# jby1993/SelfReconCode

Measured on AMD Instinct MI355X. Metric: train.py-equivalent iterations/sec (540x540, 2048 rays/frame x 3 frames per GPU; coarse stage at Adam lr 0.0001), higher is better.
Workload: dtype f32

## Files before the change

### include/selfrecon_hip.h

```cpp
#ifndef SELFRECON_HIP_H_
#define SELFRECON_HIP_H_
#include <stdint.h>

#ifdef __cplusplus
extern "C" {
#endif

#define SR_OK 0
#define SR_EINVAL (-1)
#define SR_ELAUNCH (-2)
#define SR_ENOSPC (-3)

int sr_abi_version(void);
const char* sr_build_arch(void);
const char* sr_build_digest(void);

int sr_minv3x3_fwd_f32(const float* ms, float* invs, uint8_t* checks, int64_t n, void* stream);
int sr_minv3x3_fwd_f64(const double* ms, double* invs, uint8_t* checks, int64_t n, void* stream);
int sr_minv3x3_bwd_f32(const float* grads, const float* invs, float* outs, int64_t n, void* stream);
int sr_minv3x3_bwd_f64(const double* grads, const double* invs, double* outs, int64_t n, void* stream);

typedef struct {
  int64_t size[5];
  int64_t stride[5];
// ... 64 lines not shown
  const float* Z; int64_t ldz;
  const float* A; int64_t lda;
  float* dW; int64_t lddw;
  float* partial;
  int32_t R, N, K, splits, accumulate;
  float* db; float* db_partial; int32_t group;
} sr_gemm_tn_args;
int64_t sr_mlp_gemm_tn_workspace_floats(int32_t R, int32_t N, int64_t lddw, int32_t* host_splits_out);
int sr_mlp_gemm_tn(const sr_gemm_tn_args* host_args, void* stream);
#define SR_TN_GROUP_MAX 12
typedef struct {
  int32_t n;
  sr_gemm_tn_args p[SR_TN_GROUP_MAX];
} sr_gemm_tn_group_args;
int sr_mlp_gemm_tn_group(const sr_gemm_tn_group_args* host_args, void* stream);

int sr_pe_embed(const float* x, int64_t P, int32_t L, const float* band_weights, const float* extra, int64_t ldextra,
                int32_t E, const int64_t* extra_index , int32_t group, float* out, int64_t ldo, void* stream);
int sr_pe_embed_bwd(const float* x, int64_t P, int32_t L, const float* band_weights, int32_t group, const float* gA0,
                    int64_t ldg, float* xbar, void* stream);

typedef struct {
  const float* p; const float* tp; int64_t P;
  const float* A; const float* trans; int32_t nframes;
  const int64_t* batch_inds; int64_t points_per_frame;
  const float* vol; int32_t D, H, W;
  float bmin[3], bmax[3];
  float* y;
  float* jac;
} sr_lbs_args;
// ... 195 lines not shown
```

### selfreconcode_amd/_lib.py

```python
import ctypes
import os
import torch

from .build import LIB

_i64, _vp, _int = ctypes.c_int64, ctypes.c_void_p, ctypes.c_int


class SrTensor5(ctypes.Structure):
    _fields_ = [("size", _i64 * 5), ("stride", _i64 * 5)]


class SrGemmArgs(ctypes.Structure):
    _fields_ = [("A", _vp), ("lda", _i64), ("B", _vp), ("ldb", _i64), ("C", _vp), ("ldc", _i64),
                ("M", ctypes.c_int32), ("N", ctypes.c_int32), ("K", ctypes.c_int32), ("bias", _vp),
                ("group", ctypes.c_int32), ("act", ctypes.c_int32), ("mode", ctypes.c_int32), ("out_scale", ctypes.c_float),
                ("aux", _vp), ("ldaux", _i64), ("naux_fwd", ctypes.c_int32), ("nact_bwd", ctypes.c_int32),
                ("aux_scale", ctypes.c_float)]


class SrGemmTnArgs(ctypes.Structure):
    _fields_ = [("Z", _vp), ("ldz", _i64), ("A", _vp), ("lda", _i64), ("dW", _vp), ("lddw", _i64), ("partial", _vp),
                ("R", ctypes.c_int32), ("N", ctypes.c_int32), ("K", ctypes.c_int32), ("splits", ctypes.c_int32),
                ("accumulate", ctypes.c_int32), ("db", _vp), ("db_partial", _vp), ("group", ctypes.c_int32)]
# ... 124 lines not shown
    "sr_gridsample3d_fwd_f64": [_vp, _T5, _vp, _T5, _vp, _T5, _vp],
    "sr_gridsample3d_bwd_f32": [_vp, _T5, _vp, _T5, _vp, _T5, _vp, _T5, _vp, _vp],
    "sr_gridsample3d_bwd_f64": [_vp, _T5, _vp, _T5, _vp, _T5, _vp, _T5, _vp, _vp],
    "sr_gridsample3d_dbwd_f32": [_vp, _T5, _vp, _T5, _vp, _T5, _vp, _T5, _vp, _T5, _vp, _T5, _vp, _vp, _vp],
    "sr_gridsample3d_dbwd_f64": [_vp, _T5, _vp, _T5, _vp, _T5, _vp, _T5, _vp, _T5, _vp, _T5, _vp, _vp, _vp],
    "sr_mlp_gemm_nt": [_vp, _vp],
    "sr_mlp_gemm_nt_tile": [ctypes.c_int32, ctypes.c_int32, _vp, _vp],
    "sr_mlp_chain": [_vp, _vp],
    "sr_refine_init": [_vp, _vp],
    "sr_refine_embed": [_vp, ctypes.c_int32, _vp],
    "sr_refine_mid": [_vp, ctypes.c_int32, ctypes.c_int32, _vp],
    "sr_refine_finish": [_vp, ctypes.c_int32, _vp],
    "sr_mlp_gemm_tn_workspace_floats": [ctypes.c_int32, ctypes.c_int32, _i64, _vp],
    "sr_mlp_gemm_tn": [_vp, _vp],
    "sr_mlp_gemm_tn_group": [_vp, _vp],
    "sr_lbs_chain_fwd": [_vp, ctypes.c_int32, _vp, _vp, _vp, _vp, _vp, _vp],
    "sr_lbs_chain_bwd": [_vp, ctypes.c_int32, _vp, _vp, _vp, _vp, _vp, _vp, _vp],
    "sr_lbs_fwd": [_vp, _vp],
    "sr_lbs_bwd_workspace_floats": [_i64, ctypes.c_int32],
    "sr_lbs_bwd": [_vp, _vp, _vp, _vp, _vp, _vp, _vp],
    "sr_lbs_jac_bwd": [_vp, _vp, _vp, _vp, _vp, _vp, _vp, _vp],
    "sr_newton_update": [_vp, _vp],
    "sr_newton_prepare": [_vp, _vp],
    "sr_newton_apply": [_vp, _vp],
    "sr_mc_workspace_bytes": [ctypes.c_int32, ctypes.c_int32, ctypes.c_int32],
    "sr_mc_count": [_vp, ctypes.c_int32, ctypes.c_int32, ctypes.c_int32, ctypes.c_float, _vp, _vp, _vp],
    "sr_mc_emit": [_vp, ctypes.c_int32, ctypes.c_int32, ctypes.c_int32, ctypes.c_float, _vp] + [ctypes.c_float] * 6 + [_vp, _vp, _vp],
    "sr_rows_pad": [_vp, _i64, ctypes.c_int32, _vp, _i64, ctypes.c_int32, _i64, ctypes.c_int32, _vp, _i64, ctypes.c_int32, _vp],
    "sr_rows_frame_sum_workspace_floats": [_i64, ctypes.c_int32, ctypes.c_int32],
    "sr_rows_frame_sum": [_vp, _i64, _i64, ctypes.c_int32, _vp, ctypes.c_int32, _vp, _vp, _vp],
# ... 46 lines not shown
    "sr_texture_fill_workspace_bytes": [ctypes.c_int32],
    "sr_texture_fill": [_vp, _vp, _vp, ctypes.c_int32, ctypes.c_int32, _vp, _vp, _vp],
    "sr_lbsw_knn_blend": [_vp, _vp, _i64] + [ctypes.c_int32] * 5 + [_vp, _vp, ctypes.c_int32, _vp, _vp],
    "sr_lbsw_smooth": [_vp, _vp] + [ctypes.c_int32] * 4 + [_vp],
    "sr_smpl_shape": [_vp, _vp, _vp, ctypes.c_int32, ctypes.c_int32, _i64, _vp, _vp],
    "sr_smpl_regress_workspace_floats": [ctypes.c_int32, _i64, ctypes.c_int32],
    "sr_smpl_regress": [_vp, _vp, ctypes.c_int32, _i64, ctypes.c_int32, _vp, _vp, _vp],
    "sr_smpl_pose": [_vp, _vp, _vp, _vp, ctypes.c_int32, _vp, _vp, _vp, _vp],
    "sr_smpl_skin": [_vp, _i64, _vp, _vp, _vp, _vp, ctypes.c_int32, _i64, _vp, _vp],
    "sr_meshreg_workspace_bytes": [_i64, _i64],
    "sr_meshreg_fwd": [_vp, _i64, _vp, _vp, _i64, _vp, _i64, ctypes.c_int32, ctypes.c_float] + [_vp] * 6,
    "sr_meshreg_bwd": [_i64, _vp, _vp, _i64, _vp, _vp, _i64] + [_vp] * 8,
    "sr_pe_embed_bwd": [_vp, _i64, ctypes.c_int32, _vp, ctypes.c_int32, _vp, _i64, _vp, _vp],
    "sr_pe_embed": [_vp, _i64, ctypes.c_int32, _vp, _vp, _i64, ctypes.c_int32, _vp, ctypes.c_int32, _vp, _i64, _vp],
}
_RESTYPE = {"sr_rows_frame_sum_workspace_floats": _i64, "sr_lbs_bwd_workspace_floats": _i64, "sr_mlp_gemm_tn_workspace_floats": _i64, "sr_mc_workspace_bytes": _i64, "sr_points_silhouette_workspace_bytes": _i64,
            "sr_texture_fill_workspace_bytes": _i64, "sr_meshreg_workspace_bytes": _i64, "sr_smpl_regress_workspace_floats": _i64}

_fn = {}
for _name, _args in SIGNATURES.items():
    try:
        _f = getattr(_lib, _name)
    except AttributeError as e:
        raise ImportError(f"{LIB} does not export {_name}; rebuild it") from e
    _f.argtypes = _args
    _f.restype = _RESTYPE.get(_name, _int)
    _fn[_name] = _f
_lib.sr_abi_version.restype = _int
_lib.sr_build_arch.restype = ctypes.c_char_p
_lib.sr_build_digest.restype = ctypes.c_char_p

# ... 61 lines not shown
        t = t.float()
    return t if t.is_contiguous() else t.contiguous()


def i64c(t):
    t = t.detach()
    if t.dtype != torch.int64:
        t = t.long()
    return t if t.is_contiguous() else t.contiguous()


_raw_stream = getattr(torch._C, "_cuda_getCurrentRawStream", None)


def stream_of(t):
    if _raw_stream is not None and t.device.index is not None:
        return _raw_stream(t.device.index)
    return torch.cuda.current_stream(t.device).cuda_stream


class _NoContext:
    def __enter__(self):
        return self

    def __exit__(self, *exc):
        return False


_NO_CONTEXT = _NoContext()


def on_device(dev):
    if dev.index is not None and dev.index == torch.cuda.current_device():
# ... 18 lines not shown
```

### selfreconcode_amd/csrc/mlp_gemm.hip

```cpp
#include "sr_common.h"
#include <stdlib.h>
#include <type_traits>

typedef float f32x16 __attribute__((ext_vector_type(16)));
typedef float f32x4 __attribute__((ext_vector_type(4)));
typedef int i32x4 __attribute__((ext_vector_type(4)));

__device__ __forceinline__ __amdgpu_buffer_rsrc_t sr_make_rsrc(const void* base, int64_t bytes) {
  return __builtin_amdgcn_make_buffer_rsrc(const_cast<void*>(base), 0, (int)(bytes < 0xFFFFFFFFll ? bytes : 0xFFFFFFFFll), 0x00020000);
}
__device__ __forceinline__ f32x4 sr_buffer_load16(__amdgpu_buffer_rsrc_t rsrc, uint32_t lane_off, uint32_t scalar_off) {
  return __builtin_bit_cast(f32x4, __builtin_amdgcn_raw_buffer_load_b128(rsrc, (int)lane_off, (int)scalar_off, 0));
}

namespace {

constexpr int BK = 32;
constexpr int LDSP = BK + 4;

__device__ __forceinline__ float fast_exp(float x) { return __builtin_amdgcn_exp2f(x * 1.4426950408889634f); }
__device__ __forceinline__ float fast_log(float x) { return __builtin_amdgcn_logf(x) * 0.6931471805599453f; }
__device__ __forceinline__ float softplus100(float z) {
  const float t = z * 100.0f;
  const float e = fast_exp(fminf(t, 20.0f));
// ... 586 lines not shown
  int blocks[SR_TN_GROUP_MAX];
  int rows_per_split[SR_TN_GROUP_MAX];
  sr_gemm_tn_args p[SR_TN_GROUP_MAX];
};
__global__ __launch_bounds__(256) __attribute__((amdgpu_waves_per_eu(2))) void gemm_tn_group_kernel(TnGroup G) {
  extern __shared__ __attribute__((aligned(16))) float tn_smem[];
  int i = 0;
  while (i + 1 < G.n && (int)blockIdx.x >= G.first[i + 1]) ++i;
  const int bid = blockIdx.x - G.first[i];
  if (bid >= G.blocks[i]) return;
  gemm_tn_body<128, 128>(G.p[i], G.rows_per_split[i], bid, G.blocks[i], tn_smem);
}

static inline bool tn_narrow(int N, int64_t K) { return K <= 64 && N >= 256; }

__device__ __forceinline__ void slab_reduce_body(const float* __restrict__ partial, float* __restrict__ dW, int N,
                                                 int K, int64_t lddw, int splits, int accumulate,
                                                 const float* __restrict__ db_partial, float* __restrict__ db, int bid, int nblocks) {
  const int64_t total = (int64_t)N * lddw;
  const int64_t quads = total >> 2;
  const int64_t all = quads + (db ? N : 0);
  const f32x4* __restrict__ p4 = reinterpret_cast<const f32x4*>(partial);
  f32x4* __restrict__ d4 = reinterpret_cast<f32x4*>(dW);
  for (int64_t i = (int64_t)bid * blockDim.x + threadIdx.x; i < all; i += (int64_t)nblocks * blockDim.x) {
    if (i < quads) {
      const int col = (int)((i << 2) % lddw);
      f32x4 s = {0.f, 0.f, 0.f, 0.f};
      if (col < K) {
        const f32x4* src = p4 + i;
        int p = 0;
        for (; p + 8 <= splits; p += 8) {
          f32x4 v[8];
#pragma unroll
          for (int j = 0; j < 8; ++j) v[j] = src[(int64_t)(p + j) * quads];
#pragma unroll
          for (int j = 0; j < 8; ++j) s += v[j];
        }
        for (; p < splits; ++p) s += src[(int64_t)p * quads];
        if (col + 1 >= K) s.y = 0.f;
        if (col + 2 >= K) s.z = 0.f;
        if (col + 3 >= K) s.w = 0.f;
      }
      f32x4 o = {0.f, 0.f, 0.f, 0.f};
      if (accumulate) o = d4[i];
      d4[i] = o + s;
    } else {
      const int n = (int)(i - quads);
      float s = 0.f;
      for (int p = 0; p < splits; ++p) s += db_partial[(int64_t)p * N + n];
      db[n] = (accumulate ? db[n] : 0.f) + s;
    }
  }
}

__global__ __launch_bounds__(256) void slab_reduce_kernel(const float* __restrict__ partial, float* __restrict__ dW, int N,
                                                           int K, int64_t lddw, int splits, int accumulate,
                                                           const float* __restrict__ db_partial, float* __restrict__ db) {
  slab_reduce_body(partial, dW, N, K, lddw, splits, accumulate, db_partial, db, blockIdx.x, gridDim.x);
}

__global__ __launch_bounds__(256) void slab_reduce_group_kernel(TnGroup G) {
  int i = 0;
  while (i + 1 < G.n && (int)blockIdx.x >= G.first[i + 1]) ++i;
  const int bid = blockIdx.x - G.first[i];
  if (bid >= G.blocks[i]) return;
  const sr_gemm_tn_args& g = G.p[i];
  slab_reduce_body(g.partial, g.dW, g.N, g.K, g.lddw, g.R > 0 ? g.splits : 0, g.accumulate, g.db_partial, g.db, bid, G.blocks[i]);
}

}

static void nt_tile_choice(int M, int ncols, int* bm, int* bn) {
  auto cost = [&](int tm, int tn, double eff) {
    const int64_t wgs = sr_cdiv(M, tm) * sr_cdiv(ncols, tn);
    return (double)sr_cdiv(wgs, 256) * tm * tn / eff;
  };
  if (ncols <= 32) {
    const double c[3] = {cost(32, 32, 0.6), cost(64, 32, 0.8), cost(256, 32, 1.0)};
    *bn = 32;
    if (c[0] < c[1] && c[0] < c[2]) *bm = 32;
    else if (c[1] < c[2]) *bm = 64;
    else *bm = 256;
// ... 91 lines not shown
  }
  return sr_launch_status();
}

int64_t sr_mlp_gemm_tn_workspace_floats(int32_t R, int32_t N, int64_t lddw, int32_t* splits_out) {
  const int tiles = tn_narrow(N, lddw) ? (int)sr_cdiv(N, 256) : (int)(sr_cdiv(N, 128) * sr_cdiv(lddw, 128));
  const int target = 512;
  int splits = (int)sr_cdiv(target, tiles);
  const int max_splits = (int)sr_cdiv(R, 384);
  if (splits > max_splits) splits = max_splits;
  if (splits < 1) splits = 1;
  if (splits_out) *splits_out = splits;
  return (int64_t)splits * N * lddw;
}

int sr_mlp_gemm_tn(const sr_gemm_tn_args* a, void* stream) {
  if (!a || !a->dW || !a->partial || a->R < 0 || a->N <= 0 || a->K <= 0 || a->splits < 1) return SR_EINVAL;
  if (a->R > 0 && (!a->Z || !a->A)) return SR_EINVAL;
  if ((a->ldz & 3) || (a->lda & 3) || ((uintptr_t)a->Z & 15) || ((uintptr_t)a->A & 15) || a->lddw < a->K) return SR_EINVAL;
  if ((a->lddw & 3) || ((uintptr_t)a->dW & 15) || ((uintptr_t)a->partial & 15)) return SR_EINVAL;
  if ((a->db != nullptr) != (a->db_partial != nullptr) || (a->db && a->group < 1)) return SR_EINVAL;
  const bool narrow = tn_narrow(a->N, a->lddw);
  const int tiles = narrow ? (int)sr_cdiv(a->N, 256) : (int)(sr_cdiv(a->N, 128) * sr_cdiv(a->K, 128));
  int rows_per_split = (int)sr_cdiv(a->R, a->splits);
  rows_per_split = (int)(sr_cdiv(rows_per_split, TBR) * TBR);
  if (a->R > 0) {
    using Narrow = TnCfg<256, 64>;
    using Square = TnCfg<128, 128>;
    if (narrow)
      hipLaunchKernelGGL((gemm_tn_kernel<256, 64>), dim3(tiles * a->splits), dim3(256), Narrow::kLdsFloats * sizeof(float), (hipStream_t)stream, *a,
                         rows_per_split);
    else
      hipLaunchKernelGGL((gemm_tn_kernel<128, 128>), dim3(tiles * a->splits), dim3(256), Square::kLdsFloats * sizeof(float), (hipStream_t)stream, *a,
                         rows_per_split);
  }
  const int64_t total = (int64_t)a->N * a->lddw / 4 + (a->db ? a->N : 0);
  hipLaunchKernelGGL(slab_reduce_kernel, dim3(sr_stream_grid(total, 256)), dim3(256), 0, (hipStream_t)stream, a->partial, a->dW,
                     a->N, a->K, a->lddw, a->R > 0 ? a->splits : 0, a->accumulate, a->db_partial, a->db);
  return sr_launch_status();
}

static int tn_check(const sr_gemm_tn_args* a) {
  if (!a || !a->dW || !a->partial || a->R < 0 || a->N <= 0 || a->K <= 0 || a->splits < 1) return SR_EINVAL;
  if (a->R > 0 && (!a->Z || !a->A)) return SR_EINVAL;
  if ((a->ldz & 3) || (a->lda & 3) || ((uintptr_t)a->Z & 15) || ((uintptr_t)a->A & 15) || a->lddw < a->K) return SR_EINVAL;
  if ((a->lddw & 3) || ((uintptr_t)a->dW & 15) || ((uintptr_t)a->partial & 15)) return SR_EINVAL;
  if ((a->db != nullptr) != (a->db_partial != nullptr) || (a->db && a->group < 1)) return SR_EINVAL;
  return SR_OK;
}

int sr_mlp_gemm_tn_group(const sr_gemm_tn_group_args* a, void* stream) {
  if (!a || a->n < 1 || a->n > SR_TN_GROUP_MAX) return SR_EINVAL;
  TnGroup G, Rd;
  G.n = Rd.n = a->n;
  int nb = 0, nr = 0;
  bool any_rows = false;
  for (int i = 0; i < a->n; ++i) {
    const sr_gemm_tn_args& p = a->p[i];
    const int rc = tn_check(&p);
    if (rc != SR_OK) return rc;
    if (tn_narrow(p.N, p.lddw)) return SR_EINVAL;
    const int tiles = (int)(sr_cdiv(p.N, 128) * sr_cdiv(p.K, 128));
    int rows_per_split = (int)sr_cdiv(p.R, p.splits);
    rows_per_split = (int)(sr_cdiv(rows_per_split, TBR) * TBR);
    G.p[i] = Rd.p[i] = p;
    G.rows_per_split[i] = Rd.rows_per_split[i] = rows_per_split;
    G.first[i] = nb; G.blocks[i] = p.R > 0 ? tiles * p.splits : 0;
    nb += (int)(sr_cdiv(G.blocks[i], 8) * 8);
    const int64_t total = (int64_t)p.N * p.lddw / 4 + (p.db ? p.N : 0);
    Rd.first[i] = nr; Rd.blocks[i] = sr_stream_grid(total, 256);
    nr += Rd.blocks[i];
    any_rows = any_rows || p.R > 0;
  }
  G.first[a->n] = nb; Rd.first[a->n] = nr;
  using Square = TnCfg<128, 128>;
  if (any_rows && nb > 0)
    hipLaunchKernelGGL(gemm_tn_group_kernel, dim3(nb), dim3(256), Square::kLdsFloats * sizeof(float), (hipStream_t)stream, G);
  hipLaunchKernelGGL(slab_reduce_group_kernel, dim3(nr), dim3(256), 0, (hipStream_t)stream, Rd);
  return sr_launch_status();
}
}

namespace {
__global__ __launch_bounds__(256) void pe_embed_kernel(const float* __restrict__ x, int64_t P, int L, const float* __restrict__ w,
                                                        const float* __restrict__ extra, int64_t ldextra, int E,
                                                        const int64_t* __restrict__ extra_index, int group,
                                                        float* __restrict__ out, int64_t ldo) {
  const int width = 3 + 6 * L + E;
  const int64_t total = P * ldo;
  for (int64_t i = (int64_t)blockIdx.x * blockDim.x + threadIdx.x; i < total; i += (int64_t)gridDim.x * blockDim.x) {
    const int64_t p = i / ldo;
    const int c = (int)(i % ldo);
    float v = 0.f, t3[3] = {0.f, 0.f, 0.f};
// ... 68 lines not shown
```

### selfreconcode_amd/mlp_engine.py

```python
import collections
import contextlib
import ctypes
import math
import os
import weakref
import torch

from . import _lib

ACT_NONE, ACT_SOFTPLUS100, ACT_RELU = 0, 1, 2
EPI_FWD, EPI_BWD = 0, 1

TN_SIDE_STREAM = True
GROUP_TN_BELOW = 16384
DEBUG_TN_DELAY_MS = int(os.environ.get("SR_DEBUG_TN_DELAY_MS", "0"))
_TN_STREAMS = {}
_TN_PENDING = set()
_DELAY_FLAG = {}

DEFERRED_PARAM_GRADS = False

_PACK_CACHE = {}
_ENTRY_BY_PTR = {}

_INPUT_GRADS_ONLY = False


def pad4(n):
    return (n + 3) // 4 * 4


# ... 22 lines not shown
                layers.append(LayerSpec(k, n - K0, ACT_SOFTPLUS100, 1.0 / math.sqrt(2.0), nfill=K0))
            else:
                layers.append(LayerSpec(k, n, ACT_NONE if last else ACT_SOFTPLUS100))
            k = n
        return MLPSpec(layers, K0)

    @staticmethod
    def relu_mlp(K0, widths):
        layers, k = [], K0
        for i, n in enumerate(widths):
            layers.append(LayerSpec(k, n, ACT_NONE if i == len(widths) - 1 else ACT_RELU))
            k = n
        return MLPSpec(layers, K0)


_GemmRecord = collections.namedtuple("_GemmRecord", "e0 e1 flop rows overlap N K mode group")


class _GemmProfile:

    def __init__(self):
        self.overlap = False
        self.reset(enabled=False)

    def reset(self, enabled, reserve=0):
        self.enabled = enabled
        self.records, self.chains, self.pool = [], [], []
        for _ in range(reserve if enabled else 0):
            e0, e1 = torch.cuda.Event(enable_timing=True), torch.cuda.Event(enable_timing=True)
            e0.record(); e1.record()
            self.pool.append((e0, e1))

    def pair(self):
        return self.pool.pop() if self.pool else (torch.cuda.Event(enable_timing=True), torch.cuda.Event(enable_timing=True))

    def launch(self, name, args, stream, timed=True, what=None, marks=None):
        if not (timed and self.enabled):
            _lib.call(name, ctypes.byref(args), stream)
            return
        e0, e1 = self.pair()
        e0.record()
        _lib.call(name, ctypes.byref(args), stream)
        e1.record()
        if marks is not None:
            marks.append((e0, e1) + what)
        else:
            rows, N, K, mode, group = what
            self.records.append(_GemmRecord(e0, e1, 2.0 * rows * N * K, rows, self.overlap, N, K, mode, group))

    def summary(self):
        if not self.records:
            return {"tflops": 0.0, "launches": 0, "avg_us": 0.0, "avg_flop": 0.0}
        torch.cuda.synchronize()
        for marks, live, overlap in self.chains:
            lv = live.tolist()
            for e0, e1, phase, fpr in marks:
                self.records.append(_GemmRecord(e0, e1, fpr * lv[phase], lv[phase], overlap, 0, 0, "chain", 1))
        self.chains = []
        times = [r.e0.elapsed_time(r.e1) for r in self.records]

        def rate(sel):
            f = sum(r.flop for r, t, k in zip(self.records, times, sel) if k)
            ms = sum(t for t, k in zip(times, sel) if k)
            n = sum(1 for k in sel if k)
            return (f / (ms * 1e-3) / 1e12 if ms > 0 else 0.0), n, (ms * 1e3 / n if n else 0.0), (f / n if n else 0.0)

        nt = [r.mode != "tn" for r in self.records]
        alone = [k and not r.overlap for k, r in zip(nt, self.records)]
        tf, n, us, fl = rate(alone)
        tf_all, n_all, us_all, _ = rate(nt)
        tf_big, n_big, _, _ = rate([a and r.rows >= 65536 for a, r in zip(alone, self.records)])
        tf_tn, n_tn, us_tn, _ = rate([not k for k in nt])
        self._times = times
        f_nt = float(sum(r.flop for r, k in zip(self.records, nt) if k))
        f_tn = float(sum(r.flop for r, k in zip(self.records, nt) if not k))
        return {"tflops": round(tf, 3), "launches": n, "avg_us": round(us, 3), "avg_flop": round(fl, 1), "tflops_large": round(tf_big, 3),
                "launches_large": n_big, "tflops_all": round(tf_all, 3), "launches_all": n_all, "avg_us_all": round(us_all, 3),
                "avg_flop_all": round(f_nt / max(n_all, 1), 1), "flops_total": f_nt, "flops_total_tn": f_tn,
                "tflops_tn": round(tf_tn, 3), "launches_tn": n_tn, "avg_us_tn": round(us_tn, 3)}

    def by_shape(self):
        if not self.records:
            return []
        times = getattr(self, "_times", None) or [r.e0.elapsed_time(r.e1) for r in self.records]
        acc = {}
        for r, t in zip(self.records, times):
            a = acc.setdefault((r.rows, r.N, r.K, r.mode, r.group, bool(r.overlap)), [0, 0.0, 0.0])
            a[0] += 1; a[1] += r.flop; a[2] += t
        rows = [{"M": k[0], "N": k[1], "K": k[2], "mode": k[3], "group": k[4], "overlap": k[5], "launches": v[0], "flop": v[1], "ms": round(v[2], 4),
                 "tflops": round(v[1] / (v[2] * 1e-3) / 1e12, 2) if v[2] > 0 else 0.0} for k, v in acc.items()]
        rows.sort(key=lambda r: -r["ms"])
        return rows


PROFILE = _GemmProfile()


def set_gemm_args(a, A, B, C, M, N, K, bias, group, act, mode, out_scale=1.0, aux=None, naux_fwd=0, nact_bwd=0, aux_scale=1.0, pitches=None):
    lda, ldb, ldc, ldaux = pitches or (A.stride(0), B.stride(0), C.stride(0), 0 if aux is None else aux.stride(0))
# ... 14 lines not shown
_TnProblem = collections.namedtuple("_TnProblem", "Z ldz A lda R N K lddw group dW db accumulate")


def _tn_workspace(R, N, lddw):
    splits = ctypes.c_int32(0)
    ws = _lib.raw("sr_mlp_gemm_tn_workspace_floats")(R, N, lddw, ctypes.byref(splits))
    return max(int(ws), 1), splits.value


def _set_tn_args(a, Z, ldz, A, lda, R, N, K, lddw, group, dW, db, accumulate, partial, ws, splits):
    a.Z, a.ldz, a.A, a.lda, a.dW, a.lddw, a.partial = Z.data_ptr(), ldz, A.data_ptr(), lda, dW.data_ptr(), lddw, partial
    a.R, a.N, a.K, a.splits, a.accumulate = R, N, K, splits, 1 if accumulate else 0
    a.db, a.db_partial, a.group = db.data_ptr(), partial + 4 * ws, group


def _gemm_tn(Z, ldz, A, lda, R, N, K, lddw, group=1, dW=None, db=None, accumulate=False):
    ws, splits = _tn_workspace(R, N, lddw)
    if dW is None:
        dW = torch.empty((N, lddw), dtype=torch.float32, device=Z.device)
    partial = torch.empty((ws + splits * N,), dtype=torch.float32, device=Z.device)
    if db is None:
        db = torch.empty((N,), dtype=torch.float32, device=Z.device)
    a = _lib.SrGemmTnArgs()
    _set_tn_args(a, Z, ldz, A, lda, R, N, K, lddw, group, dW, db, accumulate, partial.data_ptr(), ws, splits)
    PROFILE.launch("sr_mlp_gemm_tn", a, _lib.stream_of(Z), R >= 128 and N > 32, (R, N, K, "tn", group))
    return dW, db


def _tn_is_narrow(N, lddw):
    return lddw <= 64 and N >= 256


def _gemm_tn_group(problems):
    problems = [_TnProblem(*p) for p in problems]
    g = _lib.SrGemmTnGroupArgs()
    g.n = len(problems)
    sizes, total = [], 0
    for p in problems:
        ws, splits = _tn_workspace(p.R, p.N, p.lddw)
        sizes.append((ws, splits, total))
        total += (ws + splits * p.N + 3) // 4 * 4
    partial = torch.empty((total,), dtype=torch.float32, device=problems[0].Z.device)
    for a, p, (ws, splits, off) in zip(g.p, problems, sizes):
        _set_tn_args(a, *p, partial.data_ptr() + 4 * off, ws, splits)
    _lib.call("sr_mlp_gemm_tn_group", ctypes.byref(g), _lib.stream_of(partial))


def _debug_delay(device, ms):
    f = _DELAY_FLAG.get(str(device))
# ... 6 lines not shown
    key = str(device)
    st = _TN_STREAMS.get(key)
    if st is None:
        st = _TN_STREAMS[key] = torch.cuda.Stream(device=device)
    return st


def _launch_on_tn_stream(device, problems):
    main, side = torch.cuda.current_stream(device), _tn_stream(device)
    ready = torch.cuda.Event()
    ready.record(main)
    side.wait_event(ready)
    with torch.cuda.stream(side):
        if DEBUG_TN_DELAY_MS:
            _debug_delay(device, DEBUG_TN_DELAY_MS)
        if len(problems) == 1:
            p = problems[0]
            _gemm_tn(*p[:9], dW=p.dW, db=p.db, accumulate=p.accumulate)
        else:
            _gemm_tn_group(problems)
    for p in problems:
        p.Z.record_stream(side); p.A.record_stream(side)
    _TN_PENDING.add(str(device))


def join_weight_gradient_stream():
    for key in list(_TN_PENDING):
        st = _TN_STREAMS[key]
        torch.cuda.current_stream(st.device).wait_stream(st)
    _TN_PENDING.clear()


def _check_mat(t, name):
    if t.dtype != torch.float32 or not t.is_cuda or t.dim() != 2 or t.stride(1) != 1 or (t.stride(0) % 4) or (t.data_ptr() % 16):
        raise RuntimeError(f"mlp_engine: {name} must be a GPU fp32 matrix with unit column stride, row pitch % 4 == 0 "
                           f"and 16-byte alignment (got {tuple(t.shape)}, strides {t.stride()}, {t.dtype}, {t.device})")


def _bias_segments(b0, R, group):
    if b0 is None or b0.dim() != 2:
        return None
# ... 47 lines not shown
    if TN_SIDE_STREAM and not PROFILE.enabled:
        return _DW_SIDE, sink
    return _DW_SINK, sink


def reverse(spec, A0, WTs, acts, Ybar, group, need_input_grad=True, need_param_grad=True, Ws=None, bs=None):
    _check_mat(Ybar, "Ybar")
    R = A0.shape[0]
    nl = len(spec.layers)
    dWs, dbs = [None] * nl, [None] * nl
    A0bar_extra = None
    Zbar = Ybar
    A0bar = None
    seg = _bias_segments(bs[0], R, group) if bs is not None else None
    grouped = [] if (0 < R < GROUP_TN_BELOW and TN_SIDE_STREAM and not PROFILE.enabled) else None
    with _lib.on_device(A0.device):
        for l in range(nl - 1, -1, -1):
            L = spec.layers[l]
            X = A0 if l == 0 else acts[l - 1]
            if need_param_grad:
                route, sink = _weight_gradient_route(l, L, Ws, bs, seg, grouped)
                if sink is not None:
                    p = _TnProblem(Zbar, Zbar.stride(0), X, X.stride(0), R, L.N, L.K, pad4(L.K), group, *sink)
                    if route == _DW_GROUPED:
                        grouped.append(p)
                    elif route == _DW_SIDE:
                        _launch_on_tn_stream(A0.device, [p])
                    else:
                        _gemm_tn(*p[:9], dW=p.dW, db=p.db, accumulate=p.accumulate)
                elif route == _DW_SEGMENTED:
                    S, rs = seg
                    dWs[0] = torch.empty((L.N, pad4(L.K)), dtype=torch.float32, device=A0.device)
                    dbs[0] = torch.zeros((S, L.N), dtype=torch.float32, device=A0.device)
                    for s in range(S):
                        _gemm_tn(Zbar[s * rs:(s + 1) * rs], Zbar.stride(0), X[s * rs:(s + 1) * rs], X.stride(0), rs, L.N, L.K, pad4(L.K), group,
                                 dW=dWs[0], db=dbs[0][s], accumulate=s > 0)
                else:
                    dWs[l], dbs[l] = _gemm_tn(Zbar, Zbar.stride(0), X, X.stride(0), R, L.N, L.K, pad4(L.K), group)
            if l > 0:
                Pv = spec.layers[l - 1]
                Znew = torch.empty((R, pad4(L.K)), dtype=torch.float32, device=A0.device)
                _gemm_nt(Zbar, Zbar.stride(0), WTs[l], WTs[l].stride(0), Znew, Znew.stride(0), R, L.K, L.N, None, group, Pv.act,
                         EPI_BWD, out_scale=Pv.out_scale, aux=acts[l - 1], ldaux=acts[l - 1].stride(0), nact_bwd=Pv.N,
                         aux_scale=Pv.out_scale)
                if Pv.nfill and need_input_grad:
                    A0bar_extra = Znew[:, Pv.N:Pv.N + Pv.nfill]
                Zbar = Znew
            elif need_input_grad:
                A0bar = torch.empty((R, pad4(L.K)), dtype=torch.float32, device=A0.device)
                _gemm_nt(Zbar, Zbar.stride(0), WTs[0], WTs[0].stride(0), A0bar, A0bar.stride(0), R, L.K, L.N, None, 1, ACT_NONE,
                         EPI_FWD)
                if A0bar_extra is not None:
                    A0bar[:, :A0bar_extra.shape[1]] += A0bar_extra
        if grouped:
            _launch_on_tn_stream(A0.device, grouped)
    return A0bar, dWs, dbs


def transpose_padded(W, K):
    N = W.shape[0]
    WT = torch.zeros((K, pad4(N)), dtype=W.dtype, device=W.device)
    WT[:, :N] = W[:, :K].t()
    return WT


def pad_cols(t, width):
    if t.shape[1] == width and t.is_contiguous():
        return t
    return torch.nn.functional.pad(t, (0, width - t.shape[1]))

# ... 390 lines not shown
```

Measured before the change: 23.49.

## Defer weight-gradient slab reductions and batch them into one multi-problem reduce kernel

```diff
diff --git a/include/selfrecon_hip.h b/include/selfrecon_hip.h
--- a/include/selfrecon_hip.h
+++ b/include/selfrecon_hip.h
@@ -102,6 +102,10 @@
   sr_gemm_tn_args p[SR_TN_GROUP_MAX];
 } sr_gemm_tn_group_args;
 int sr_mlp_gemm_tn_group(const sr_gemm_tn_group_args* host_args, void* stream);
+int sr_mlp_gemm_tn_tiles(const sr_gemm_tn_args* host_problems, int32_t n, void* stream);
+int64_t sr_mlp_slab_reduce_many_table_bytes(int32_t n);
+int sr_mlp_slab_reduce_many(const sr_gemm_tn_args* host_problems, int32_t n, void* table_host, void* table_dev, int64_t table_bytes,
+                            void* stream);
 
 int sr_pe_embed(const float* x, int64_t P, int32_t L, const float* band_weights, const float* extra, int64_t ldextra,
                 int32_t E, const int64_t* extra_index , int32_t group, float* out, int64_t ldo, void* stream);
diff --git a/selfreconcode_amd/_lib.py b/selfreconcode_amd/_lib.py
--- a/selfreconcode_amd/_lib.py
+++ b/selfreconcode_amd/_lib.py
@@ -162,6 +162,9 @@
     "sr_mlp_gemm_tn_workspace_floats": [ctypes.c_int32, ctypes.c_int32, _i64, _vp],
     "sr_mlp_gemm_tn": [_vp, _vp],
     "sr_mlp_gemm_tn_group": [_vp, _vp],
+    "sr_mlp_gemm_tn_tiles": [_vp, ctypes.c_int32, _vp],
+    "sr_mlp_slab_reduce_many_table_bytes": [ctypes.c_int32],
+    "sr_mlp_slab_reduce_many": [_vp, ctypes.c_int32, _vp, _vp, _i64, _vp],
     "sr_lbs_chain_fwd": [_vp, ctypes.c_int32, _vp, _vp, _vp, _vp, _vp, _vp],
     "sr_lbs_chain_bwd": [_vp, ctypes.c_int32, _vp, _vp, _vp, _vp, _vp, _vp, _vp],
     "sr_lbs_fwd": [_vp, _vp],
@@ -238,7 +241,8 @@
     "sr_pe_embed_bwd": [_vp, _i64, ctypes.c_int32, _vp, ctypes.c_int32, _vp, _i64, _vp, _vp],
     "sr_pe_embed": [_vp, _i64, ctypes.c_int32, _vp, _vp, _i64, ctypes.c_int32, _vp, ctypes.c_int32, _vp, _i64, _vp],
 }
-_RESTYPE = {"sr_rows_frame_sum_workspace_floats": _i64, "sr_lbs_bwd_workspace_floats": _i64, "sr_mlp_gemm_tn_workspace_floats": _i64, "sr_mc_workspace_bytes": _i64, "sr_points_silhouette_workspace_bytes": _i64,
+_RESTYPE = {"sr_rows_frame_sum_workspace_floats": _i64, "sr_lbs_bwd_workspace_floats": _i64, "sr_mlp_gemm_tn_workspace_floats": _i64, "sr_mlp_slab_reduce_many_table_bytes": _i64,
+            "sr_mc_workspace_bytes": _i64, "sr_points_silhouette_workspace_bytes": _i64,
             "sr_texture_fill_workspace_bytes": _i64, "sr_meshreg_workspace_bytes": _i64, "sr_smpl_regress_workspace_floats": _i64}
 
 _fn = {}
@@ -330,9 +334,13 @@
 
 
 def stream_of(t):
-    if _raw_stream is not None and t.device.index is not None:
-        return _raw_stream(t.device.index)
-    return torch.cuda.current_stream(t.device).cuda_stream
+    return stream_of_device(t.device)
+
+
+def stream_of_device(device):
+    if _raw_stream is not None and device.index is not None:
+        return _raw_stream(device.index)
+    return torch.cuda.current_stream(device).cuda_stream
 
 
 class _NoContext:
diff --git a/selfreconcode_amd/csrc/mlp_gemm.hip b/selfreconcode_amd/csrc/mlp_gemm.hip
--- a/selfreconcode_amd/csrc/mlp_gemm.hip
+++ b/selfreconcode_amd/csrc/mlp_gemm.hip
@@ -1,6 +1,9 @@
 #include "sr_common.h"
 #include <stdlib.h>
+#include <algorithm>
 #include <type_traits>
+#include <utility>
+#include <vector>
 
 typedef float f32x16 __attribute__((ext_vector_type(16)));
 typedef float f32x4 __attribute__((ext_vector_type(4)));
@@ -624,6 +627,26 @@
 
 static inline bool tn_narrow(int N, int64_t K) { return K <= 64 && N >= 256; }
 
+__device__ __forceinline__ f32x4 slab_sum_quad(const f32x4* __restrict__ p4, int64_t i, int64_t quads, int splits, int col, int K) {
+  f32x4 s = {0.f, 0.f, 0.f, 0.f};
+  if (col < K) {
+    const f32x4* src = p4 + i;
+    int p = 0;
+    for (; p + 8 <= splits; p += 8) {
+      f32x4 v[8];
+#pragma unroll
+      for (int j = 0; j < 8; ++j) v[j] = src[(int64_t)(p + j) * quads];
+#pragma unroll
+      for (int j = 0; j < 8; ++j) s += v[j];
+    }
+    for (; p < splits; ++p) s += src[(int64_t)p * quads];
+    if (col + 1 >= K) s.y = 0.f;
+    if (col + 2 >= K) s.z = 0.f;
+    if (col + 3 >= K) s.w = 0.f;
+  }
+  return s;
+}
+
 __device__ __forceinline__ void slab_reduce_body(const float* __restrict__ partial, float* __restrict__ dW, int N,
                                                  int K, int64_t lddw, int splits, int accumulate,
                                                  const float* __restrict__ db_partial, float* __restrict__ db, int bid, int nblocks) {
@@ -634,23 +657,7 @@
   f32x4* __restrict__ d4 = reinterpret_cast<f32x4*>(dW);
   for (int64_t i = (int64_t)bid * blockDim.x + threadIdx.x; i < all; i += (int64_t)nblocks * blockDim.x) {
     if (i < quads) {
-      const int col = (int)((i << 2) % lddw);
-      f32x4 s = {0.f, 0.f, 0.f, 0.f};
-      if (col < K) {
-        const f32x4* src = p4 + i;
-        int p = 0;
-        for (; p + 8 <= splits; p += 8) {
-          f32x4 v[8];
-#pragma unroll
-          for (int j = 0; j < 8; ++j) v[j] = src[(int64_t)(p + j) * quads];
-#pragma unroll
-          for (int j = 0; j < 8; ++j) s += v[j];
-        }
-        for (; p < splits; ++p) s += src[(int64_t)p * quads];
-        if (col + 1 >= K) s.y = 0.f;
-        if (col + 2 >= K) s.z = 0.f;
-        if (col + 3 >= K) s.w = 0.f;
-      }
+      const f32x4 s = slab_sum_quad(p4, i, quads, splits, (int)((i << 2) % lddw), K);
       f32x4 o = {0.f, 0.f, 0.f, 0.f};
       if (accumulate) o = d4[i];
       d4[i] = o + s;
@@ -676,6 +683,59 @@
   if (bid >= G.blocks[i]) return;
   const sr_gemm_tn_args& g = G.p[i];
   slab_reduce_body(g.partial, g.dW, g.N, g.K, g.lddw, g.R > 0 ? g.splits : 0, g.accumulate, g.db_partial, g.db, bid, G.blocks[i]);
+}
+
+struct ReduceEntry {
+  const float* partial; float* dW; const float* db_partial; float* db;
+  int64_t quads, lddw;
+  int32_t N, K, splits, accumulate;
+};
+struct ReduceChain {
+  int64_t quads;
+  int32_t first_block, nblocks, first_entry, n_entries, db_n, pad_;
+};
+__global__ __launch_bounds__(256) void slab_reduce_many_kernel(const ReduceChain* __restrict__ chains, int nchains, const ReduceEntry* __restrict__ entries) {
+  int lo = 0, hi = nchains - 1;
+  while (lo < hi) {
+    const int mid = (lo + hi + 1) >> 1;
+    if (chains[mid].first_block <= (int)blockIdx.x) lo = mid; else hi = mid - 1;
+  }
+  const ReduceChain ch = chains[lo];
+  const int bid = blockIdx.x - ch.first_block;
+  if (bid >= ch.nblocks) return;
+  const ReduceEntry* __restrict__ ent = entries + ch.first_entry;
+  const int64_t all = ch.quads + ch.db_n;
+  for (int64_t i = (int64_t)bid * blockDim.x + threadIdx.x; i < all; i += (int64_t)ch.nblocks * blockDim.x) {
+    if (i < ch.quads) {
+      for (int e = 0; e < ch.n_entries; ++e) {
+        const ReduceEntry& g = ent[e];
+        if (i >= g.quads) continue;
+        const f32x4 s = slab_sum_quad(reinterpret_cast<const f32x4*>(g.partial), i, g.quads, g.splits, (int)((i << 2) % g.lddw), g.K);
+        f32x4* d4 = reinterpret_cast<f32x4*>(g.dW);
+        f32x4 o = {0.f, 0.f, 0.f, 0.f};
+        if (g.accumulate) o = d4[i];
+        d4[i] = o + s;
+      }
+    } else {
+      const int n = (int)(i - ch.quads);
+      for (int e = 0; e < ch.n_entries; ++e) {
+        const ReduceEntry& g = ent[e];
+        if (!g.db || n >= g.N) continue;
+        float s = 0.f;
+        for (int p = 0; p < g.splits; ++p) s += g.db_partial[(int64_t)p * g.N + n];
+        g.db[n] = (g.accumulate ? g.db[n] : 0.f) + s;
+      }
+    }
+  }
+}
+
+struct Span { uintptr_t lo, hi; int owner; uintptr_t base; };
+template <class F>
+bool spans_clash(const std::vector<Span>& v, F allowed) {
+  for (size_t i = 0; i < v.size(); ++i)
+    for (size_t j = i + 1; j < v.size(); ++j)
+      if (v[i].lo < v[j].hi && v[j].lo < v[i].hi && !allowed(v[i], v[j])) return true;
+  return false;
 }
 
 }
@@ -797,32 +857,6 @@
   return (int64_t)splits * N * lddw;
 }
 
-int sr_mlp_gemm_tn(const sr_gemm_tn_args* a, void* stream) {
-  if (!a || !a->dW || !a->partial || a->R < 0 || a->N <= 0 || a->K <= 0 || a->splits < 1) return SR_EINVAL;
-  if (a->R > 0 && (!a->Z || !a->A)) return SR_EINVAL;
-  if ((a->ldz & 3) || (a->lda & 3) || ((uintptr_t)a->Z & 15) || ((uintptr_t)a->A & 15) || a->lddw < a->K) return SR_EINVAL;
-  if ((a->lddw & 3) || ((uintptr_t)a->dW & 15) || ((uintptr_t)a->partial & 15)) return SR_EINVAL;
-  if ((a->db != nullptr) != (a->db_partial != nullptr) || (a->db && a->group < 1)) return SR_EINVAL;
-  const bool narrow = tn_narrow(a->N, a->lddw);
-  const int tiles = narrow ? (int)sr_cdiv(a->N, 256) : (int)(sr_cdiv(a->N, 128) * sr_cdiv(a->K, 128));
-  int rows_per_split = (int)sr_cdiv(a->R, a->splits);
-  rows_per_split = (int)(sr_cdiv(rows_per_split, TBR) * TBR);
-  if (a->R > 0) {
-    using Narrow = TnCfg<256, 64>;
-    using Square = TnCfg<128, 128>;
-    if (narrow)
-      hipLaunchKernelGGL((gemm_tn_kernel<256, 64>), dim3(tiles * a->splits), dim3(256), Narrow::kLdsFloats * sizeof(float), (hipStream_t)stream, *a,
-                         rows_per_split);
-    else
-      hipLaunchKernelGGL((gemm_tn_kernel<128, 128>), dim3(tiles * a->splits), dim3(256), Square::kLdsFloats * sizeof(float), (hipStream_t)stream, *a,
-                         rows_per_split);
-  }
-  const int64_t total = (int64_t)a->N * a->lddw / 4 + (a->db ? a->N : 0);
-  hipLaunchKernelGGL(slab_reduce_kernel, dim3(sr_stream_grid(total, 256)), dim3(256), 0, (hipStream_t)stream, a->partial, a->dW,
-                     a->N, a->K, a->lddw, a->R > 0 ? a->splits : 0, a->accumulate, a->db_partial, a->db);
-  return sr_launch_status();
-}
-
 static int tn_check(const sr_gemm_tn_args* a) {
   if (!a || !a->dW || !a->partial || a->R < 0 || a->N <= 0 || a->K <= 0 || a->splits < 1) return SR_EINVAL;
   if (a->R > 0 && (!a->Z || !a->A)) return SR_EINVAL;
@@ -832,34 +866,174 @@
   return SR_OK;
 }
 
-int sr_mlp_gemm_tn_group(const sr_gemm_tn_group_args* a, void* stream) {
-  if (!a || a->n < 1 || a->n > SR_TN_GROUP_MAX) return SR_EINVAL;
-  TnGroup G, Rd;
-  G.n = Rd.n = a->n;
+static void tn_launch_tiles(const sr_gemm_tn_args* a, void* stream) {
+  if (a->R <= 0) return;
+  const bool narrow = tn_narrow(a->N, a->lddw);
+  const int tiles = narrow ? (int)sr_cdiv(a->N, 256) : (int)(sr_cdiv(a->N, 128) * sr_cdiv(a->K, 128));
+  int rows_per_split = (int)sr_cdiv(a->R, a->splits);
+  rows_per_split = (int)(sr_cdiv(rows_per_split, TBR) * TBR);
+  using Narrow = TnCfg<256, 64>;
+  using Square = TnCfg<128, 128>;
+  if (narrow)
+    hipLaunchKernelGGL((gemm_tn_kernel<256, 64>), dim3(tiles * a->splits), dim3(256), Narrow::kLdsFloats * sizeof(float), (hipStream_t)stream, *a,
+                       rows_per_split);
+  else
+    hipLaunchKernelGGL((gemm_tn_kernel<128, 128>), dim3(tiles * a->splits), dim3(256), Square::kLdsFloats * sizeof(float), (hipStream_t)stream, *a,
+                       rows_per_split);
+}
+
+static int tn_launch_tiles_group(const sr_gemm_tn_args* p_in, int n, void* stream, TnGroup* Rd, int* nr_out) {
+  TnGroup G;
+  G.n = n;
+  if (Rd) Rd->n = n;
   int nb = 0, nr = 0;
   bool any_rows = false;
-  for (int i = 0; i < a->n; ++i) {
-    const sr_gemm_tn_args& p = a->p[i];
+  for (int i = 0; i < n; ++i) {
+    const sr_gemm_tn_args& p = p_in[i];
     const int rc = tn_check(&p);
     if (rc != SR_OK) return rc;
     if (tn_narrow(p.N, p.lddw)) return SR_EINVAL;
     const int tiles = (int)(sr_cdiv(p.N, 128) * sr_cdiv(p.K, 128));
     int rows_per_split = (int)sr_cdiv(p.R, p.splits);
     rows_per_split = (int)(sr_cdiv(rows_per_split, TBR) * TBR);
-    G.p[i] = Rd.p[i] = p;
-    G.rows_per_split[i] = Rd.rows_per_split[i] = rows_per_split;
+    G.p[i] = p;
+    G.rows_per_split[i] = rows_per_split;
     G.first[i] = nb; G.blocks[i] = p.R > 0 ? tiles * p.splits : 0;
     nb += (int)(sr_cdiv(G.blocks[i], 8) * 8);
-    const int64_t total = (int64_t)p.N * p.lddw / 4 + (p.db ? p.N : 0);
-    Rd.first[i] = nr; Rd.blocks[i] = sr_stream_grid(total, 256);
-    nr += Rd.blocks[i];
+    if (Rd) {
+      const int64_t total = (int64_t)p.N * p.lddw / 4 + (p.db ? p.N : 0);
+      Rd->p[i] = p; Rd->rows_per_split[i] = rows_per_split;
+      Rd->first[i] = nr; Rd->blocks[i] = sr_stream_grid(total, 256);
+      nr += Rd->blocks[i];
+    }
     any_rows = any_rows || p.R > 0;
   }
-  G.first[a->n] = nb; Rd.first[a->n] = nr;
+  G.first[n] = nb;
+  if (Rd) { Rd->first[n] = nr; *nr_out = nr; }
   using Square = TnCfg<128, 128>;
   if (any_rows && nb > 0)
     hipLaunchKernelGGL(gemm_tn_group_kernel, dim3(nb), dim3(256), Square::kLdsFloats * sizeof(float), (hipStream_t)stream, G);
+  return SR_OK;
+}
+
+int sr_mlp_gemm_tn(const sr_gemm_tn_args* a, void* stream) {
+  const int rc = tn_check(a);
+  if (rc != SR_OK) return rc;
+  tn_launch_tiles(a, stream);
+  const int64_t total = (int64_t)a->N * a->lddw / 4 + (a->db ? a->N : 0);
+  hipLaunchKernelGGL(slab_reduce_kernel, dim3(sr_stream_grid(total, 256)), dim3(256), 0, (hipStream_t)stream, a->partial, a->dW,
+                     a->N, a->K, a->lddw, a->R > 0 ? a->splits : 0, a->accumulate, a->db_partial, a->db);
+  return sr_launch_status();
+}
+
+int sr_mlp_gemm_tn_group(const sr_gemm_tn_group_args* a, void* stream) {
+  if (!a || a->n < 1 || a->n > SR_TN_GROUP_MAX) return SR_EINVAL;
+  TnGroup Rd;
+  int nr = 0;
+  const int rc = tn_launch_tiles_group(a->p, a->n, stream, &Rd, &nr);
+  if (rc != SR_OK) return rc;
   hipLaunchKernelGGL(slab_reduce_group_kernel, dim3(nr), dim3(256), 0, (hipStream_t)stream, Rd);
+  return sr_launch_status();
+}
+
+int sr_mlp_gemm_tn_tiles(const sr_gemm_tn_args* p, int32_t n, void* stream) {
+  if (!p || n < 1 || n > SR_TN_GROUP_MAX) return SR_EINVAL;
+  if (n == 1) {
+    const int rc = tn_check(p);
+    if (rc != SR_OK) return rc;
+    tn_launch_tiles(p, stream);
+  } else {
+    const int rc = tn_launch_tiles_group(p, n, stream, nullptr, nullptr);
+    if (rc != SR_OK) return rc;
+  }
+  return sr_launch_status();
+}
+
+int64_t sr_mlp_slab_reduce_many_table_bytes(int32_t n) {
+  if (n < 0) return SR_EINVAL;
+  return (int64_t)n * (int64_t)(sizeof(ReduceChain) + sizeof(ReduceEntry));
+}
+
+int sr_mlp_slab_reduce_many(const sr_gemm_tn_args* p, int32_t n, void* table_host, void* table_dev, int64_t table_bytes, void* stream) {
+  if (n == 0) return SR_OK;
+  if (!p || n < 0 || !table_host || !table_dev || table_bytes < sr_mlp_slab_reduce_many_table_bytes(n)) return SR_EINVAL;
+  if (((uintptr_t)table_host & 15) || ((uintptr_t)table_dev & 15)) return SR_EINVAL;
+  for (int i = 0; i < n; ++i) {
+    const sr_gemm_tn_args& a = p[i];
+    if (!a.dW || !a.partial || a.R < 0 || a.N <= 0 || a.K <= 0 || a.splits < 1 || a.lddw < a.K) return SR_EINVAL;
+    if ((a.lddw & 3) || ((uintptr_t)a.dW & 15) || ((uintptr_t)a.partial & 15)) return SR_EINVAL;
+    if ((a.db != nullptr) != (a.db_partial != nullptr) || ((uintptr_t)a.db & 3) || ((uintptr_t)a.db_partial & 3)) return SR_EINVAL;
+  }
+  std::vector<Span> part, dws, dbs, mixed;
+  for (int i = 0; i < n; ++i) {
+    const sr_gemm_tn_args& a = p[i];
+    const uintptr_t pl = (uintptr_t)a.partial, dl = (uintptr_t)a.dW;
+    part.push_back({pl, pl + (uintptr_t)a.splits * a.N * a.lddw * 4, i, pl});
+    dws.push_back({dl, dl + (uintptr_t)a.N * a.lddw * 4, i, dl});
+    if (a.db) {
+      const uintptr_t bl = (uintptr_t)a.db_partial, ol = (uintptr_t)a.db;
+      part.push_back({bl, bl + (uintptr_t)a.splits * a.N * 4, i, bl});
+      dbs.push_back({ol, ol + (uintptr_t)a.N * 4, i, ol});
+    }
+  }
+  auto both_dst = [&](const Span& x, const Span& y) { return x.owner >= n && y.owner >= n; };
+  mixed = part;
+  for (Span s : dws) { s.owner += n; mixed.push_back(s); }
+  for (Span s : dbs) { s.owner += n; mixed.push_back(s); }
+  if (spans_clash(mixed, both_dst)) return SR_EINVAL;
+  auto same_dw = [&](const Span& x, const Span& y) { return x.base == y.base && p[x.owner].lddw == p[y.owner].lddw; };
+  auto same_db = [&](const Span& x, const Span& y) { return x.base == y.base && p[x.owner].dW == p[y.owner].dW; };
+  auto dw_db = [&](const Span& x, const Span& y) { return (x.owner >= n) == (y.owner >= n); };
+  mixed = dws;
+  for (Span s : dbs) { s.owner += n; mixed.push_back(s); }
+  if (spans_clash(dws, same_dw) || spans_clash(dbs, same_db) || spans_clash(mixed, dw_db)) return SR_EINVAL;
+
+  std::vector<std::vector<int>> members;
+  {
+    std::vector<std::pair<uintptr_t, int>> seen;
+    for (int i = 0; i < n; ++i) {
+      int c = -1;
+      for (const auto& s : seen) if (s.first == (uintptr_t)p[i].dW) { c = s.second; break; }
+      if (c < 0) { c = (int)members.size(); members.emplace_back(); seen.push_back({(uintptr_t)p[i].dW, c}); }
+      members[c].push_back(i);
+    }
+  }
+  const int nchains = (int)members.size();
+  ReduceChain* chains = (ReduceChain*)table_host;
+  ReduceEntry* entries = (ReduceEntry*)((char*)table_host + (size_t)n * sizeof(ReduceChain));
+  std::vector<int64_t> full(nchains);
+  std::vector<double> weight(nchains);
+  int64_t full_sum = 0; double weight_sum = 0;
+  int ne = 0;
+  for (int c = 0; c < nchains; ++c) {
+    ReduceChain& ch = chains[c];
+    ch.quads = 0; ch.db_n = 0; ch.first_entry = ne; ch.n_entries = (int)members[c].size(); ch.pad_ = 0;
+    weight[c] = 0;
+    for (int i : members[c]) {
+      const sr_gemm_tn_args& a = p[i];
+      ReduceEntry& e = entries[ne++];
+      e.partial = a.partial; e.dW = a.dW; e.db_partial = a.db_partial; e.db = a.db;
+      e.quads = (int64_t)a.N * a.lddw / 4; e.lddw = a.lddw;
+      e.N = a.N; e.K = a.K; e.splits = a.R > 0 ? a.splits : 0; e.accumulate = a.accumulate;
+      ch.quads = std::max(ch.quads, e.quads);
+      if (a.db) ch.db_n = std::max(ch.db_n, a.N);
+      weight[c] += (double)e.quads * (e.splits + 1);
+    }
+    full[c] = sr_cdiv(ch.quads + ch.db_n, 256);
+    full_sum += full[c]; weight_sum += weight[c];
+  }
+  const int64_t kGrid = 2048;
+  int64_t nb = 0;
+  for (int c = 0; c < nchains; ++c) {
+    int64_t b = full[c];
+    if (full_sum > kGrid) b = std::min<int64_t>(full[c], std::max<int64_t>(1, (int64_t)(kGrid * (weight[c] / weight_sum) + 0.5)));
+    chains[c].first_block = (int)nb; chains[c].nblocks = (int)b;
+    nb += b;
+  }
+  const size_t bytes = (size_t)n * (sizeof(ReduceChain) + sizeof(ReduceEntry));
+  if (hipMemcpyAsync(table_dev, table_host, bytes, hipMemcpyHostToDevice, (hipStream_t)stream) != hipSuccess) return SR_ELAUNCH;
+  hipLaunchKernelGGL(slab_reduce_many_kernel, dim3((unsigned)nb), dim3(256), 0, (hipStream_t)stream, (const ReduceChain*)table_dev, nchains,
+                     (const ReduceEntry*)((const char*)table_dev + (size_t)n * sizeof(ReduceChain)));
   return sr_launch_status();
 }
 }
diff --git a/selfreconcode_amd/mlp_engine.py b/selfreconcode_amd/mlp_engine.py
--- a/selfreconcode_amd/mlp_engine.py
+++ b/selfreconcode_amd/mlp_engine.py
@@ -14,7 +14,10 @@
 TN_SIDE_STREAM = True
 GROUP_TN_BELOW = 16384
 DEBUG_TN_DELAY_MS = int(os.environ.get("SR_DEBUG_TN_DELAY_MS", "0"))
+TN_REDUCE_AT = "sweep"
+TN_PENDING_BYTES_MAX = 1 << 30
 _TN_STREAMS = {}
+_TN_LISTS = {}
 _TN_PENDING = set()
 _DELAY_FLAG = {}
 
@@ -67,7 +70,14 @@
         return MLPSpec(layers, K0)
 
 
-_GemmRecord = collections.namedtuple("_GemmRecord", "e0 e1 flop rows overlap N K mode group")
+_GemmRecord = collections.namedtuple("_GemmRecord", "e0 e1 flop rows overlap N K mode group extra", defaults=(None,))
+
+
+def _record_ms(r):
+    ms = r.e0.elapsed_time(r.e1)
+    for e0, e1, share in r.extra or ():
+        ms += share * e0.elapsed_time(e1)
+    return ms
 
 
 class _GemmProfile:
@@ -88,18 +98,20 @@
         return self.pool.pop() if self.pool else (torch.cuda.Event(enable_timing=True), torch.cuda.Event(enable_timing=True))
 
     def launch(self, name, args, stream, timed=True, what=None, marks=None):
+        lead = args if isinstance(args, tuple) else (ctypes.byref(args),)
         if not (timed and self.enabled):
-            _lib.call(name, ctypes.byref(args), stream)
-            return
+            _lib.call(name, *lead, stream)
+            return None
         e0, e1 = self.pair()
         e0.record()
-        _lib.call(name, ctypes.byref(args), stream)
+        _lib.call(name, *lead, stream)
         e1.record()
         if marks is not None:
             marks.append((e0, e1) + what)
-        else:
-            rows, N, K, mode, group = what
-            self.records.append(_GemmRecord(e0, e1, 2.0 * rows * N * K, rows, self.overlap, N, K, mode, group))
+            return None
+        rows, N, K, mode, group = what
+        self.records.append(_GemmRecord(e0, e1, 2.0 * rows * N * K, rows, self.overlap, N, K, mode, group, [] if mode == "tn" else None))
+        return self.records[-1]
 
     def summary(self):
         if not self.records:
@@ -110,7 +122,7 @@
             for e0, e1, phase, fpr in marks:
                 self.records.append(_GemmRecord(e0, e1, fpr * lv[phase], lv[phase], overlap, 0, 0, "chain", 1))
         self.chains = []
-        times = [r.e0.elapsed_time(r.e1) for r in self.records]
+        times = [_record_ms(r) for r in self.records]
 
         def rate(sel):
             f = sum(r.flop for r, t, k in zip(self.records, times, sel) if k)
@@ -135,7 +147,7 @@
     def by_shape(self):
         if not self.records:
             return []
-        times = getattr(self, "_times", None) or [r.e0.elapsed_time(r.e1) for r in self.records]
+        times = getattr(self, "_times", None) or [_record_ms(r) for r in self.records]
         acc = {}
         for r, t in zip(self.records, times):
             a = acc.setdefault((r.rows, r.N, r.K, r.mode, r.group, bool(r.overlap)), [0, 0.0, 0.0])
@@ -180,13 +192,106 @@
     a.db, a.db_partial, a.group = db.data_ptr(), partial + 4 * ws, group
 
 
-def _gemm_tn(Z, ldz, A, lda, R, N, K, lddw, group=1, dW=None, db=None, accumulate=False):
-    ws, splits = _tn_workspace(R, N, lddw)
+class _TnPendingList:
+    __slots__ = ("device", "stream", "raw", "args", "keep", "records", "bytes", "ws", "used", "want", "high", "old_ws", "tables")
+
+    def __init__(self, device, stream, raw):
+        self.device, self.stream, self.raw = device, stream, raw
+        self.args, self.keep, self.records, self.bytes = [], [], [], 0
+        self.ws, self.used, self.old_ws = None, 0, []
+        self.want, self.high = 0, 0
+        self.tables = collections.deque()
+
+    def take(self, nfloats):
+        nfloats = (nfloats + 3) // 4 * 4
+        self.want += nfloats
+        if self.ws is None or self.used + nfloats > self.ws.numel():
+            if self.ws is not None and self.used:
+                self.old_ws.append(self.ws)
+            cap = max(self.want, self.high, 2 * self.ws.numel() if self.ws is not None else 0)
+            self.ws, self.used = torch.empty((cap,), dtype=torch.float32, device=self.device), 0
+        ptr = self.ws.data_ptr() + 4 * self.used
+        self.used += nfloats
+        return ptr
+
+    def add(self, a, nbytes, dW, db, record):
+        self.args.append(a); self.keep.append((dW, db)); self.records.append((record, nbytes))
+        self.bytes += nbytes
+
+    def _table(self, nbytes):
+        while self.tables and self.tables[0][0].query():
+            t = self.tables.popleft()[1]
+            if t.numel() >= nbytes:
+                return t
+        return torch.empty((max(nbytes, 4096),), dtype=torch.uint8, pin_memory=True)
+
+    def reduce(self):
+        n = len(self.args)
+        if n == 0:
+            return
+        with _lib.on_device(self.device), (_lib._NO_CONTEXT if _lib.stream_of_device(self.device) == self.raw else torch.cuda.stream(self.stream)):
+            arr = (_lib.SrGemmTnArgs * n)(*self.args)
+            nbytes = int(_lib.raw("sr_mlp_slab_reduce_many_table_bytes")(n))
+            host = self._table(nbytes)
+            dev = torch.empty((nbytes,), dtype=torch.uint8, device=self.device)
+            timed = PROFILE.enabled and any(r is not None for r, _ in self.records)
+            if timed:
+                e0, e1 = PROFILE.pair()
+                e0.record()
+            _lib.call("sr_mlp_slab_reduce_many", arr, n, host.data_ptr(), dev.data_ptr(), nbytes, self.raw)
+            if timed:
+                e1.record()
+                for r, b in self.records:
+                    if r is not None:
+                        r.extra.append((e0, e1, b / self.bytes))
+            done = torch.cuda.Event()
+            done.record()
+            self.tables.append((done, host))
+        self.args, self.keep, self.records, self.bytes = [], [], [], 0
+        self.used, self.old_ws = 0, []
+        self.high, self.want = max(self.high, self.want), 0
+        if self.ws is not None and self.high > self.ws.numel():
+            self.ws = None
+
+
+def _pending_list(device):
+    raw = _lib.stream_of_device(device)
+    lst = _TN_LISTS.get((device.index, raw))
+    if lst is None:
+        lst = _TN_LISTS[(device.index, raw)] = _TnPendingList(device, torch.cuda.current_stream(device), raw)
+    return lst
+
+
+def reduce_pending_weight_gradients():
+    for lst in _TN_LISTS.values():
+        lst.reduce()
+
+
+def _tn_defer(pending, problems, structs):
+    need = [_tn_workspace(p.R, p.N, p.lddw) for p in problems]
+    nbytes = [4 * (ws + splits * p.N) for p, (ws, splits) in zip(problems, need)]
+    if pending.args and pending.bytes + sum(nbytes) > TN_PENDING_BYTES_MAX:
+        pending.reduce()
+    for a, p, (ws, splits) in zip(structs, problems, need):
+        _set_tn_args(a, *p, pending.take(ws + splits * p.N), ws, splits)
+    p0 = problems[0]
+    timed = len(problems) == 1 and p0.R >= 128 and p0.N > 32
+    rec = PROFILE.launch("sr_mlp_gemm_tn_tiles", (structs, len(problems)), pending.raw, timed, (p0.R, p0.N, p0.K, "tn", p0.group))
+    for a, p, b in zip(structs, problems, nbytes):
+        pending.add(a, b, p.dW, p.db, rec)
+
+
+def _gemm_tn(Z, ldz, A, lda, R, N, K, lddw, group=1, dW=None, db=None, accumulate=False, pending=None):
     if dW is None:
         dW = torch.empty((N, lddw), dtype=torch.float32, device=Z.device)
-    partial = torch.empty((ws + splits * N,), dtype=torch.float32, device=Z.device)
     if db is None:
         db = torch.empty((N,), dtype=torch.float32, device=Z.device)
+    if pending is not None:
+        arr = (_lib.SrGemmTnArgs * 1)()
+        _tn_defer(pending, [_TnProblem(Z, ldz, A, lda, R, N, K, lddw, group, dW, db, accumulate)], arr)
+        return dW, db
+    ws, splits = _tn_workspace(R, N, lddw)
+    partial = torch.empty((ws + splits * N,), dtype=torch.float32, device=Z.device)
     a = _lib.SrGemmTnArgs()
     _set_tn_args(a, Z, ldz, A, lda, R, N, K, lddw, group, dW, db, accumulate, partial.data_ptr(), ws, splits)
     PROFILE.launch("sr_mlp_gemm_tn", a, _lib.stream_of(Z), R >= 128 and N > 32, (R, N, K, "tn", group))
@@ -197,8 +302,11 @@
     return lddw <= 64 and N >= 256
 
 
-def _gemm_tn_group(problems):
+def _gemm_tn_group(problems, pending=None):
     problems = [_TnProblem(*p) for p in problems]
+    if pending is not None:
+        _tn_defer(pending, problems, (_lib.SrGemmTnArgs * len(problems))())
+        return
     g = _lib.SrGemmTnGroupArgs()
     g.n = len(problems)
     sizes, total = [], 0
@@ -235,17 +343,20 @@
     with torch.cuda.stream(side):
         if DEBUG_TN_DELAY_MS:
             _debug_delay(device, DEBUG_TN_DELAY_MS)
+        pending = _pending_list(device)
         if len(problems) == 1:
             p = problems[0]
-            _gemm_tn(*p[:9], dW=p.dW, db=p.db, accumulate=p.accumulate)
+            _gemm_tn(*p[:9], dW=p.dW, db=p.db, accumulate=p.accumulate, pending=pending)
         else:
-            _gemm_tn_group(problems)
+            _gemm_tn_group(problems, pending=pending)
     for p in problems:
         p.Z.record_stream(side); p.A.record_stream(side)
     _TN_PENDING.add(str(device))
+    return pending
 
 
 def join_weight_gradient_stream():
+    reduce_pending_weight_gradients()
     for key in list(_TN_PENDING):
         st = _TN_STREAMS[key]
         torch.cuda.current_stream(st.device).wait_stream(st)
@@ -323,7 +434,10 @@
     A0bar = None
     seg = _bias_segments(bs[0], R, group) if bs is not None else None
     grouped = [] if (0 < R < GROUP_TN_BELOW and TN_SIDE_STREAM and not PROFILE.enabled) else None
+    here, side = None, None
     with _lib.on_device(A0.device):
+        if need_param_grad:
+            here = _pending_list(A0.device)
         for l in range(nl - 1, -1, -1):
             L = spec.layers[l]
             X = A0 if l == 0 else acts[l - 1]
@@ -334,18 +448,18 @@
                     if route == _DW_GROUPED:
                         grouped.append(p)
                     elif route == _DW_SIDE:
-                        _launch_on_tn_stream(A0.device, [p])
+                        side = _launch_on_tn_stream(A0.device, [p])
                     else:
-                        _gemm_tn(*p[:9], dW=p.dW, db=p.db, accumulate=p.accumulate)
+                        _gemm_tn(*p[:9], dW=p.dW, db=p.db, accumulate=p.accumulate, pending=here)
                 elif route == _DW_SEGMENTED:
                     S, rs = seg
                     dWs[0] = torch.empty((L.N, pad4(L.K)), dtype=torch.float32, device=A0.device)
                     dbs[0] = torch.zeros((S, L.N), dtype=torch.float32, device=A0.device)
                     for s in range(S):
                         _gemm_tn(Zbar[s * rs:(s + 1) * rs], Zbar.stride(0), X[s * rs:(s + 1) * rs], X.stride(0), rs, L.N, L.K, pad4(L.K), group,
-                                 dW=dWs[0], db=dbs[0][s], accumulate=s > 0)
+                                 dW=dWs[0], db=dbs[0][s], accumulate=s > 0, pending=here)
                 else:
-                    dWs[l], dbs[l] = _gemm_tn(Zbar, Zbar.stride(0), X, X.stride(0), R, L.N, L.K, pad4(L.K), group)
+                    dWs[l], dbs[l] = _gemm_tn(Zbar, Zbar.stride(0), X, X.stride(0), R, L.N, L.K, pad4(L.K), group, pending=here)
             if l > 0:
                 Pv = spec.layers[l - 1]
                 Znew = torch.empty((R, pad4(L.K)), dtype=torch.float32, device=A0.device)
@@ -362,7 +476,11 @@
                 if A0bar_extra is not None:
                     A0bar[:, :A0bar_extra.shape[1]] += A0bar_extra
         if grouped:
-            _launch_on_tn_stream(A0.device, grouped)
+            side = _launch_on_tn_stream(A0.device, grouped)
+        if here is not None:
+            here.reduce()
+        if side is not None and TN_REDUCE_AT == "sweep":
+            side.reduce()
     return A0bar, dWs, dbs
 
 
```

Result: no change. 23.47 (-0.1%).
